# Fool-Yang/AlphaSnake-Zero

Measured on AMD Instinct MI355X. Metric: self-play env-steps/sec (11x11, 4 snakes, 50 MCTS sims), higher is better.
Workload: dtype f32 (tower convolutions: each f32 operand split into f16 hi + lo, 3 f16 MFMAs per product, f32 accumulate)

## Files before the change

### __graft_entry__.py

```python
import os
import subprocess
import sys

REPO = os.path.dirname(os.path.abspath(__file__))
PKG = os.path.join(REPO, "alphasnake-zero_amd")
for p in (REPO, PKG):
    if p not in sys.path:
        sys.path.insert(0, p)


def build():
    env = dict(os.environ)
    subprocess.check_call(["make", "-C", os.path.join(PKG, "csrc"), "-j4"], env=env)
    subprocess.check_call(["make", "-C", os.path.join(REPO, "oracle")], env=env)
    import snake_engine
    snake_engine.lib()
    import utils.game, utils.mp_game_runner, utils.agent, utils.alpha_nnet
    sys.path.insert(0, os.path.join(REPO, "tools"))
    import store_hazard_scan
    if os.path.exists(os.path.join(store_hazard_scan.LLVM_BIN, "llvm-objdump")):
        r = store_hazard_scan.scan_library(snake_engine.LIB_PATH)
        if r["violations"]:
            raise RuntimeError(f"{len(r['violations'])} wide store(s) whose data registers are rewritten inside the hazard window, e.g. "
                               f"{r['violations'][0]}")
# ... 23 lines not shown
    spawned = eng.new((n,), torch.int16, 0)
    for t in range(12):
        mv = rng.randint(0, 3, size=(n, 4)).astype(np.uint8)
        eng.step(torch.as_tensor(mv, device="cuda"), spawned=spawned)
        sp = spawned.cpu().numpy()
        for g in range(n):
            if sum(games[g].g.alive[:4]) > 1:
                games[g].tic(mv[g], spawn_cell=int(sp[g]))
    out = eng.export()
    for g in range(n):
        a, b = compact_from_state(out[g]), games[g].compact()
        for k in a:
            assert np.array_equal(a[k], b[k]), (g, k)
    alive = eng.alive().cpu().numpy()
    pairs = np.argwhere(alive).astype(np.int32)
    planes, mask, key = eng.observe_all(pairs)
    ph = planes.cpu().numpy()
    for i, (g, s) in enumerate(pairs[:256]):
        assert ph[i].tobytes() == games[g].make_state(int(s)).tobytes(), (g, s)
    from snake_engine import net
    from oracle import net_ref
    ws = net.glorot_uniform_weights((21, 21, 3), blocks=4, seed=0)
    qn = net.QNet(ws, (21, 21, 3))
    assert qn.n_rect == 6 and len(pairs) >= 64 >= qn.rect_min
    q_gpu = qn.forward(planes[:64].contiguous(), mask[:64].contiguous()).cpu().numpy()
    q_cpu = net_ref.forward(ws, ph[:64])
    assert np.abs(q_gpu - q_cpu).max() <= 1e-5, np.abs(q_gpu - q_cpu).max()
    from utils.agent import Agent
    from utils.alpha_nnet import AlphaNNet
    from utils.mp_game_runner import MPGameRunner
    MPGameRunner.verbose = False
    alice = Agent(AlphaNNet(input_shape=(21, 21, 3), _weights=ws), 2, True, 8, 8, seed=1)
    gr = MPGameRunner(11, 11, 4, 1, 4, seed=2)
    gr.run(alice, max_turns=1)
    assert gr.env_steps == 4 and len(alice.records) == 16 and np.isfinite(np.array(alice.values[:16])).all()
    print(f"smoke ok: {n} games x 12 ticks + {len(pairs)} observations bit-exact vs the CPU oracle; "
          f"net |dQ| = {np.abs(q_gpu - q_cpu).max():.2e}; one MCTS root turn of 4 games ({alice._mcts.stats['net_evals']} net evals)")


if __name__ == "__main__":
    build()
    if "--smoke" in sys.argv:
        smoke()
```

### alphasnake-zero_amd/csrc/conv_split.hip

```cpp
#include "common.h"
#include "train_fold.h"
#include <stdlib.h>

typedef float f32x16 __attribute__((ext_vector_type(16)));
typedef _Float16 f16x8 __attribute__((ext_vector_type(8)));
typedef _Float16 f16x4 __attribute__((ext_vector_type(4)));
typedef __bf16 bf16x8 __attribute__((ext_vector_type(8)));
typedef unsigned uint4_t __attribute__((ext_vector_type(4)));
typedef int i32x4 __attribute__((ext_vector_type(4)));
typedef int i32x8 __attribute__((ext_vector_type(8)));
typedef short s16x2 __attribute__((ext_vector_type(2)));

template <bool BF> __device__ __forceinline__ float hs_from16(_Float16 v)
{
    if (BF) return (float)__builtin_bit_cast(__bf16, v);
    return (float)v;
}
template <bool BF> __device__ __forceinline__ _Float16 hs_to16(float v)
{
    if (BF) return __builtin_bit_cast(_Float16, (__bf16)v);
    return (_Float16)__builtin_amdgcn_fmed3f(v, -65504.f, 65504.f);
}

#define HS_C 128
// ... 34 lines not shown
    const float *wscale_inv;
    const float *scale, *shift;
    const float *res;
    float *out;
    const float *w1x1;
    float *h1;
    float s1, b1;
    int Hd, Wd, n_blk, tiles_base, tiles_rem, relu;
    int n_img_grouped;
    const float *center;
    float *stat_part;
    const uint4 *desc;
    const int *n_desc;
    const float *bg_out;
    const float *bg_in;
    const float *bg_res;
    int grow_in, grow_res;
    const float *g_y;
    const unsigned char *g_mask;
    const float *g_inv;
    const float *aff_scale, *aff_shift;
    float *amax_part;
    const unsigned char *res_mask;
};

#ifdef HS_STAMPS
__device__ unsigned long long hs_stamp_buf[16384 * 8];
#define HS_STAMP(k) if (tid == 0 && blockIdx.x < 16384) hs_stamp_buf[blockIdx.x * 8 + (k)] = __builtin_amdgcn_s_memtime();
#define HS_STAMP_REAL(k) if (tid == 0 && blockIdx.x < 16384) hs_stamp_buf[blockIdx.x * 8 + (k)] = __builtin_amdgcn_s_memrealtime();
#define HS_STAMP_HWID(k) if (tid == 0 && blockIdx.x < 16384) hs_stamp_buf[blockIdx.x * 8 + (k)] = \
        (unsigned long long)__builtin_amdgcn_s_getreg((31 << 11) | 4) | (unsigned long long)__builtin_amdgcn_s_getreg((31 << 11) | 20) << 32;
__device__ unsigned long long hs_tap_buf[2048 * 8 * 10];
#define HS_TSTAMP(c_, s_) if (tid == 0 && blockIdx.x < 2048 && (c_) < 8) hs_tap_buf[(blockIdx.x * 8 + (c_)) * 10 + (s_)] = __builtin_amdgcn_s_memtime();
extern "C" int snk_dbg_conv_tap_stamps(unsigned long long *h_out)
{
    SNK_CHECK_HIP(hipMemcpyFromSymbol(h_out, HIP_SYMBOL(hs_tap_buf), sizeof(unsigned long long) * 2048 * 8 * 10));
    return 0;
}
extern "C" int snk_dbg_conv_stamps(unsigned long long *h_out, int n_blocks)
{
    SNK_CHECK_HIP(hipMemcpyFromSymbol(h_out, HIP_SYMBOL(hs_stamp_buf), (size_t)n_blocks * 8 * sizeof(unsigned long long)));
    return 0;
}
#else
#define HS_STAMP(k)
#define HS_STAMP_REAL(k)
// ... 19 lines not shown
}
__device__ __forceinline__ uint2 mx_quant8(const f16x8 v, unsigned &sbyte)
{
    const uint4 u = __builtin_bit_cast(uint4, v);
    const float f[8] = {__builtin_bit_cast(float, u.x << 16), __builtin_bit_cast(float, u.x & 0xFFFF0000u),
                        __builtin_bit_cast(float, u.y << 16), __builtin_bit_cast(float, u.y & 0xFFFF0000u),
                        __builtin_bit_cast(float, u.z << 16), __builtin_bit_cast(float, u.z & 0xFFFF0000u),
                        __builtin_bit_cast(float, u.w << 16), __builtin_bit_cast(float, u.w & 0xFFFF0000u)};
    float m = 0.f;
#pragma unroll
    for (int j = 0; j < 8; ++j) m = fmaxf(m, fabsf(f[j]));
    m = fmaxf(m, hs_dpp(m, 0xB1));
    m = fmaxf(m, hs_dpp(m, 0x4E));
    sbyte = mx_scale_byte(m);
    const float k = mx_inv_scale(sbyte);
    return make_uint2(mx_pack4(f[0] * k, f[1] * k, f[2] * k, f[3] * k), mx_pack4(f[4] * k, f[5] * k, f[6] * k, f[7] * k));
}
template <int NI, int MODE, bool SPLIT, int IO16, bool RECT, bool BF = false, bool MX = false, bool PK = false>
__device__ __forceinline__ void hs_block(const ConvHsArgs &p, unsigned char *smem, const int img, const int tile0, const int ntile,
                                         const int ry0, const int rx0, const int rh, const int rw, const unsigned bbox,
                                         const int part, const int parts, const int imgB = 0, const int ryB = 0, const int rxB = 0,
                                         const unsigned bboxB = 0u, const int nB = 0)
{
    static_assert(!PK || (RECT && SPLIT && IO16 == 0 && (MODE == 1 || MODE == 2)), "the packed form exists for the float32-accurate sub-rectangle layers only");
    static_assert(IO16 == 0 || !SPLIT, "f16 activations only exist in the reduced-precision form");
    static_assert(!BF || (IO16 & 1), "the bf16 form reads bf16 activations");
    static_assert(!MX || BF, "the mxfp8 form reads bf16 activations");
    constexpr bool IN16 = (IO16 & 1) != 0, OUT16 = (IO16 & 2) != 0;
    constexpr bool STATS = MODE == 4 || MODE == 6 || MODE == 9, GSTATS = MODE == 5 || MODE == 7 || MODE == 8 || MODE == 10, BARE = STATS || GSTATS;
    constexpr bool RESMASK = MODE == 8 || MODE == 10, AMAX = MODE == 4 || MODE == 9;
    constexpr bool AFF = MODE == 6 || MODE == 9, GAFF = MODE == 7 || MODE == 10, NORES = MODE == 7;
    static_assert(!(AFF || GAFF || RESMASK) || (SPLIT && IO16 == 0 && !RECT), "the deferred batch norm exists in the training step's float32 form only");
    constexpr bool K32 = IN16;
    constexpr int RING = K32 ? HS_RING16 : HS_RING, AHEAD = K32 ? HS_AHEAD16 : HS_AHEAD;
    constexpr bool TWO = SPLIT || K32;
    constexpr int KC = MX ? 64 : K32 ? 32 : HS_KC, NCHUNK = HS_C / KC;
    constexpr int NST = K32 ? HS_NST16 : HS_NST, BUFB = K32 ? HS_BUF16 : (PK ? HS_NPB_PK : HS_NPB) * HS_LDP;
    constexpr int PIECE = K32 ? 8 : 4;
    constexpr int MXR0_ = 9 * NI > 4 * NST ? (9 * NI - 4 * NST) / 2 : 0;
    constexpr int MXR0 = MXR0_ > HS_XLOAD_TAP * NI ? MXR0_ : HS_XLOAD_TAP * NI, MXT1 = (MXR0 + 2 * NST + NI - 1) / NI;
    constexpr int MXR1 = 9 * NI - 2 * NST > MXT1 * NI ? 9 * NI - 2 * NST : MXT1 * NI;
    constexpr bool MXIN = MX && 9 * NI >= 4 * NST && MXT1 <= 8 && MXR1 + 2 * NST <= 9 * NI;
    static_assert(!MXIN || (MXR0 >= HS_XLOAD_TAP * NI && MXR0 + 2 * NST <= MXT1 * NI), "MX staging: a half is written before it is loaded");
    constexpr bool P8 = IN16 && OUT16;
    const bool has_res = NORES ? false : RESMASK ? true : (MODE == 0 || GSTATS) ? p.res != nullptr : (MODE == 2 || MODE == 3);
    const bool has_head = MODE == 0 ? p.w1x1 != nullptr : MODE == 3;
    const bool has_out = MODE == 0 ? p.out != nullptr : MODE != 3;
// ... 567 lines not shown
            }
            v.x = fmaxf(v.x, relu_floor); v.y = fmaxf(v.y, relu_floor); v.z = fmaxf(v.z, relu_floor); v.w = fmaxf(v.w, relu_floor);
            if (STATS && off[pass & 1][j] >= 0) {
                const float ex = v.x - cen4.x, ey = v.y - cen4.y, ez = v.z - cen4.z, ew = v.w - cen4.w;
                st_s.x += ex; st_s.y += ey; st_s.z += ez; st_s.w += ew;
                st_q.x += ex * ex; st_q.y += ey * ey; st_q.z += ez * ez; st_q.w += ew * ew;
                if (AMAX) {
                    st_m.x = fmaxf(st_m.x, fabsf(ex)); st_m.y = fmaxf(st_m.y, fabsf(ey));
                    st_m.z = fmaxf(st_m.z, fabsf(ez)); st_m.w = fmaxf(st_m.w, fabsf(ew));
                }
            }
            if (has_out && off[pass & 1][j] >= 0) {
                if (OUT16) {
                    f16x4 o16_;
                    o16_[0] = hs_to16<BF>(v.x); o16_[1] = hs_to16<BF>(v.y); o16_[2] = hs_to16<BF>(v.z); o16_[3] = hs_to16<BF>(v.w);
                    *(f16x4 *)((_Float16 *)p.out + obase + off[pass & 1][j]) = o16_;
                } else *(float4 *)(p.out + obase + off[pass & 1][j]) = v;
            }
            if (has_head) {
                float d_ = (v.x * wh.x + v.y * wh.y) + (v.z * wh.z + v.w * wh.w);
                d_ += hs_dpp(d_, 0xB1); d_ += hs_dpp(d_, 0x4E); d_ += hs_dpp(d_, 0x141); d_ += hs_dpp(d_, 0x140);
                d_ += __shfl_xor(d_, 16, 64);
                if (cq == 0 && off[pass & 1][j] >= 0)
                    p.h1[(long)img * HWc + off[pass & 1][j] / HS_C] = fmaxf(__builtin_fmaf(d_, p.s1, p.b1), 0.f);
            }
        }
    }
#undef HS_ROWS
#undef HS_EPI_PREP
    if (BARE) {
        __syncthreads();
        float4 *R = (float4 *)smem;
        R[rr0 * 32 + cq] = st_s;
        R[(8 + rr0) * 32 + cq] = st_q;
        if (AMAX) R[(16 + rr0) * 32 + cq] = st_m;
        __syncthreads();
        if (AMAX && rr0 == 2 && p.amax_part) {
            float4 t = R[16 * 32 + cq];
#pragma unroll
            for (int r = 1; r < 8; ++r) {
                const float4 u = R[(16 + r) * 32 + cq];
                t.x = fmaxf(t.x, u.x); t.y = fmaxf(t.y, u.y); t.z = fmaxf(t.z, u.z); t.w = fmaxf(t.w, u.w);
            }
            *(float4 *)(p.amax_part + (size_t)blockIdx.x * HS_C + 4 * cq) = t;
        }
        if (rr0 < 2) {
            float4 t = R[(8 * rr0) * 32 + cq];
#pragma unroll
            for (int r = 1; r < 8; ++r) { const float4 u = R[(8 * rr0 + r) * 32 + cq]; t.x += u.x; t.y += u.y; t.z += u.z; t.w += u.w; }
            *(float4 *)(p.stat_part + (size_t)blockIdx.x * 256 + rr0 * 128 + 4 * cq) = t;
        }
    }
    if (PK && p.bg_out) {
        const float invF = 1.0f / (float)p.Wd;
        for (int s = 0; s < 2; ++s) {
            const int sm = s ? 0 : m0, sn = s ? nB : nA;
            if (sn == 0) continue;
            const int q_lo = (sm * HWc + HW - 1) / HW, q_hi = ((sm + sn) * HWc + HW - 1) / HW;
            const int fy = s ? ryB : cy0, fx = s ? rxB : cx0;
            float *ob = p.out + (long)(s ? imgB : img) * HWc * HS_C;
            for (int q = q_lo + rr0; q < q_hi; q += 8) {
                const int y_ = (int)(((float)q + 0.5f) * invF), x_ = q - y_ * p.Wd;
                if (y_ >= fy && y_ < fy + rh && x_ >= fx && x_ < fx + rw) continue;
                const int o_ = (y_ * p.Wd + x_) * HS_C + 4 * cq;
                *(float4 *)(ob + o_) = *(const float4 *)(p.bg_out + o_);
            }
        }
    } else if (RECT && p.bg_out) {
        const float invF = 1.0f / (float)p.Wd;
        for (int q = part * 8 + rr0; q < HWc; q += 8 * parts) {
            const int y_ = (int)(((float)q + 0.5f) * invF), x_ = q - y_ * p.Wd;
            if (y_ >= cy0 && y_ < cy0 + rh && x_ >= cx0 && x_ < cx0 + rw) continue;
            const int o_ = (y_ * p.Wd + x_) * HS_C + 4 * cq;
            if (OUT16) *(f16x4 *)((_Float16 *)p.out + (long)img * HWc * HS_C + o_) = *(const f16x4 *)((const _Float16 *)p.bg_out + o_);
            else *(float4 *)(p.out + (long)img * HWc * HS_C + o_) = *(const float4 *)(p.bg_out + o_);
        }
// ... 957 lines not shown
}

extern "C" int snk_conv3x3_bn_f16s_rect_pack(const float *d_x, const void *d_wS, const float *d_scale, const float *d_shift,
                                             const float *d_residual, float *d_out, const void *d_desc, const int *d_count,
                                             const float *d_bg_in, int grow_in, const float *d_bg_res, int grow_res,
                                             const float *d_bg_out, int n_images, int height, int width, void *stream)
{
    SNK_REQUIRE(grow_in >= 0 && grow_in < 128 && grow_res >= 0 && grow_res < 128, "snk_conv3x3_bn_f16s_rect_pack: grow_in %d, grow_res %d", grow_in, grow_res);
    SNK_REQUIRE(d_x && d_wS && d_scale && d_shift && d_out && d_desc && d_count, "snk_conv3x3_bn_f16s_rect_pack: NULL argument");
    SNK_REQUIRE(d_out != d_x, "snk_conv3x3_bn_f16s_rect_pack: in-place convolution is not possible");
    const long md = rect_pack_max_desc(n_images, height, width);
    SNK_REQUIRE(md >= 0 && md < (1l << 31) && (long)n_images * height * width * HS_C < (1l << 31), "snk_conv3x3_bn_f16s_rect_pack: bad shape %d x %d x %d",
                n_images, height, width);
    if (n_images == 0) return 0;
    ConvHsArgs a = {d_x, (const f16x8 *)d_wS, (const float *)((const _Float16 *)d_wS + HS_WS_ELEMS), d_scale, d_shift,
                    d_residual, d_out, nullptr, nullptr, 0.f, 0.f, height, width, 1, 0, 0, 1, 0, nullptr, nullptr,
                    (const uint4 *)d_desc, d_count, d_bg_out, d_bg_in, d_residual ? d_bg_res : nullptr, grow_in, grow_res, nullptr, nullptr, nullptr};
    if (d_residual) k_conv3x3_f16s_rectp<2><<<(int)(md / 2), 256, 0, (hipStream_t)stream>>>(a);
    else k_conv3x3_f16s_rectp<1><<<(int)(md / 2), 256, 0, (hipStream_t)stream>>>(a);
    SNK_CHECK_HIP(hipGetLastError());
    return 0;
}

extern "C" int snk_conv3x3_bn_f16_act16_rect(const void *d_x16, const void *d_wS, const float *d_scale, const float *d_shift,
                                             const void *d_residual16, void *d_out16, const void *d_desc, const int *d_count,
                                             const void *d_bg_in16, int grow_in, const void *d_bg_res16, int grow_res,
                                             const void *d_bg_out16, int n_images, int height, int width, void *stream)
{
    return conv_f16s_rect_launch((const float *)d_x16, d_wS, d_scale, d_shift, (const float *)d_residual16, (float *)d_out16, d_desc,
                                 d_count, (const float *)d_bg_in16, grow_in, (const float *)d_bg_res16, grow_res,
                                 (const float *)d_bg_out16, n_images, height, width, true, stream);
}

extern "C" int snk_conv3x3_bn_bf16_act16_rect(const void *d_x16, const void *d_wS, const float *d_scale, const float *d_shift,
                                              const void *d_residual16, void *d_out16, const void *d_desc, const int *d_count,
                                              const void *d_bg_in16, int grow_in, const void *d_bg_res16, int grow_res,
                                              const void *d_bg_out16, int n_images, int height, int width, void *stream)
{
    return conv_f16s_rect_launch((const float *)d_x16, d_wS, d_scale, d_shift, (const float *)d_residual16, (float *)d_out16, d_desc,
                                 d_count, (const float *)d_bg_in16, grow_in, (const float *)d_bg_res16, grow_res,
                                 (const float *)d_bg_out16, n_images, height, width, true, stream, true);
}

extern "C" int snk_conv3x3_bn_f16s(const float *d_x, const void *d_wS, const float *d_scale, const float *d_shift,
                                   const float *d_residual, float *d_out, int n_images, int height, int width, int relu,
                                   void *stream)
// ... 221 lines not shown
```

### alphasnake-zero_amd/snake_engine/_lib.py

```python
import ctypes as C
import os

_HERE = os.path.dirname(os.path.abspath(__file__))
LIB_PATH = os.environ.get("SNK_LIB_PATH") or os.path.join(_HERE, "libsnake_engine.so")

MAX_SNAKES, MAX_CELLS, MAX_NODES = 8, 361, 384
ABI_VERSION = 113


class EngineError(RuntimeError):
    pass


class SnkGameState(C.Structure):
    _fields_ = [
        ("H", C.c_int32), ("W", C.c_int32), ("S", C.c_int32), ("uid", C.c_uint32),
        ("alive", C.c_uint8 * MAX_SNAKES),
        ("health", C.c_int16 * MAX_SNAKES),
        ("length", C.c_int16 * MAX_SNAKES),
        ("dir", C.c_uint8 * MAX_SNAKES),
        ("nodes", (C.c_int16 * MAX_NODES) * MAX_SNAKES),
        ("food", C.c_uint8 * MAX_CELLS),
        ("rewards", C.c_int8 * MAX_SNAKES),
        ("counters", C.c_int32 * 6),
# ... 35 lines not shown
    "snk_conv3x3_bn_bf16_act16_head": (i32, [vp, vp, vp, vp, vp, vp, C.c_float, C.c_float, vp, i32, i32, i32, vp]),
    "snk_conv_rect_max_blocks_act16": (C.c_long, [i32, i32, i32]),
    "snk_conv_rect_plan_act16": (i32, [vp, C.c_float, C.c_float, C.c_float, i32, i32, i32, i32, C.POINTER(i32), vp, vp, vp, vp]),
    "snk_conv3x3_bn_bf16_act16": (i32, [vp, vp, vp, vp, vp, vp, i32, i32, i32, i32, i32, vp]),
    "snk_conv3x3_bn_bf16_act16_rect": (i32, [vp, vp, vp, vp, vp, vp, vp, vp, vp, i32, vp, i32, vp, i32, i32, i32, vp]),
    "snk_stem_conv_bn_relu_bf16out": (i32, [vp, vp, vp, vp, vp, i32, i32, i32, vp]),
    "snk_stem_conv_bn_relu_bf16out_rect": (i32, [vp, vp, vp, vp, vp, vp, i32, i32, i32, i32, vp]),
    "snk_conv3x3_prepare_weights_mxfp8": (i32, [vp, vp, vp]),
    "snk_conv3x3_bn_mxfp8_act16": (i32, [vp, vp, vp, vp, vp, vp, i32, i32, i32, i32, i32, vp]),
    "snk_conv3x3_bn_mxfp8_act16_rect": (i32, [vp, vp, vp, vp, vp, vp, vp, vp, vp, i32, vp, i32, vp, i32, i32, i32, vp]),
    "snk_conv3x3_bn_mxfp8_act16_head": (i32, [vp, vp, vp, vp, vp, vp, C.c_float, C.c_float, vp, i32, i32, i32, vp]),
    "snk_mxfp8_quantize_bf16": (i32, [vp, i32, vp, vp, vp]),
    "snk_conv3x3_prepare_weights_winograd": (i32, [vp, vp, vp]),
    "snk_conv3x3_bn_f32_winograd": (i32, [vp, vp, vp, vp, vp, vp, i32, i32, i32, i32, vp]),
    "snk_conv3x3_prepare_weights_f16s": (i32, [vp, vp, C.c_float, vp]),
    "snk_conv3x3_bn_f16s": (i32, [vp, vp, vp, vp, vp, vp, i32, i32, i32, i32, vp]),
    "snk_conv3x3_bn_f16": (i32, [vp, vp, vp, vp, vp, vp, i32, i32, i32, i32, vp]),
    "snk_conv_rect_max_blocks": (C.c_long, [i32, i32, i32]),
    "snk_conv_rect_plan": (i32, [vp, C.c_float, C.c_float, C.c_float, i32, i32, i32, i32, C.POINTER(i32), vp, vp, vp, vp]),
    "snk_conv_rect_pack_max_desc": (C.c_long, [i32, i32, i32]),
    "snk_conv_rect_plan_pack": (i32, [vp, C.c_float, C.c_float, C.c_float, i32, i32, i32, i32, C.POINTER(i32), vp, vp, vp, vp, vp]),
    "snk_conv_rect_plan_pack_host": (i32, [vp, i32, i32, i32, i32, vp, vp]),
    "snk_conv3x3_bn_f16s_rect_pack": (i32, [vp, vp, vp, vp, vp, vp, vp, vp, vp, i32, vp, i32, vp, i32, i32, i32, vp]),
    "snk_stem_conv_bn_relu_f32_rect": (i32, [vp, vp, vp, vp, vp, vp, i32, i32, i32, i32, vp]),
    "snk_stem_conv_bn_relu_f16out_rect": (i32, [vp, vp, vp, vp, vp, vp, i32, i32, i32, i32, vp]),
    "snk_conv3x3_bn_f16_act16_rect": (i32, [vp, vp, vp, vp, vp, vp, vp, vp, vp, i32, vp, i32, vp, i32, i32, i32, vp]),
    "snk_conv3x3_bn_f16s_rect": (i32, [vp, vp, vp, vp, vp, vp, vp, vp, vp, i32, vp, i32, vp, i32, i32, i32, vp]),
    "snk_conv3x3_bn_f16s_head": (i32, [vp, vp, vp, vp, vp, vp, vp, C.c_float, C.c_float, vp, i32, i32, i32, vp]),
    "snk_conv3x3_bn_f16_act16": (i32, [vp, vp, vp, vp, vp, vp, i32, i32, i32, i32, i32, vp]),
    "snk_stem_conv_bn_relu_f16out": (i32, [vp, vp, vp, vp, vp, i32, i32, i32, vp]),
    "snk_head_dense_f32": (i32, [vp, vp, vp, vp, vp, vp, vp, i32, i32, i32, vp]),
    "snk_stem_conv_bn_relu_f32": (i32, [vp, vp, vp, vp, vp, i32, i32, i32, vp]),
    "snk_tt_create": (i32, [C.POINTER(vp), u64, i32]),
    "snk_tt_destroy": (i32, [vp]),
    "snk_tt_clear": (i32, [vp, vp]),
    "snk_tt_status_sync": (i32, [vp, C.POINTER(C.c_int64), C.POINTER(C.c_int64), C.POINTER(i32)]),
    "snk_tt_rebuild_sync": (i32, [vp, u64, i32, i32]),
    "snk_tt_lookup_insert": (i32, [vp, vp, vp, i32, i32, i32, vp, vp, vp]),
    "snk_tt_find": (i32, [vp, vp, i32, i32, i32, vp, vp, vp]),
    "snk_tt_set_priors": (i32, [vp, vp, vp, i32, vp, vp, vp]),
    "snk_tt_read_q": (i32, [vp, vp, i32, i32, vp, vp]),
    "snk_mcts_select": (i32, [vp, vp, i32, C.c_float, vp, vp, C.c_int64, u64, C.c_uint32, C.c_uint32, vp, vp, vp, vp, vp, vp, i32, vp, vp]),
    "snk_mcts_gather_rows": (i32, [vp, i32, vp, vp, vp, vp, vp]),
    "snk_mcts_row_active": (i32, [vp, vp, i32, i32, vp, vp]),
    "snk_mcts_retire": (i32, [vp, vp, vp, i32, i32, vp, vp, vp]),
    "snk_mcts_backup": (i32, [vp, vp, i32, vp, vp, vp, vp, vp, i32, i32, vp, vp]),
# ... 86 lines not shown
```

### alphasnake-zero_amd/snake_engine/net.py

```python
import ctypes as C
import math
import os

import numpy as np
import torch

from ._lib import lib, check, EngineError

BN_EPS = 1e-3
K_FILTERS = 128
F16S_WEIGHT_BYTES = 9 * 128 * 128 * 4 + 32
F16S_TAIL_OFFSET = 9 * 128 * 128 * 4
F16S_FLAG_OFFSET = F16S_TAIL_OFFSET + 16


def glorot_uniform_weights(input_shape, blocks=4, seed=0):
    g = torch.Generator().manual_seed(seed)
    h, w, c = input_shape
    k = K_FILTERS

    def glorot(shape, fan_in, fan_out):
        lim = math.sqrt(6.0 / (fan_in + fan_out))
        return ((torch.rand(shape, generator=g, dtype=torch.float32) * 2 - 1) * lim).numpy()

# ... 70 lines not shown
    return count


class QNet:
    def __init__(self, weights, input_shape, device=None, max_chunk=4096):
        if not torch.cuda.is_available():
            raise EngineError("snake_engine.QNet needs an MI355X; there is no CPU fallback")
        self.L = lib()
        self.device = torch.device("cuda", torch.cuda.current_device() if device is None else int(device))
        self.input_shape = tuple(int(v) for v in input_shape)
        self.h, self.w, self.cin = self.input_shape
        assert self.cin == 3
        self.max_chunk = int(max_chunk)
        self._ws = None
        self.conv_timing = None
        self.clock_probe = None
        self.conv_algo = os.environ.get("SNK_CONV_ALGO", "f16s")
        if self.conv_algo not in ("f16s", "winograd", "direct", "bf16", "f16", "f16a", "mxfp8"):
            raise EngineError(f"SNK_CONV_ALGO={self.conv_algo!r}: expected f16s, winograd, direct, f16, f16a, bf16 or mxfp8")
        self.rect = self.conv_algo in ("f16s", "f16a", "bf16", "mxfp8") and os.environ.get("SNK_CONV_RECT", "1") != "0"
        self.act16 = {"f16a": torch.float16, "bf16": torch.bfloat16, "mxfp8": torch.bfloat16}.get(self.conv_algo)
        self.background = BACKGROUND_PIXEL
        self.guard_trips = 0
        self.rect_tiles = None
        self._bg = None
        self.rect_min = int(os.environ.get("SNK_CONV_RECT_MIN", "48"))
        self.rect_pack = os.environ.get("SNK_CONV_RECT_PACK", "1") != "0"
        self.n_streams = int(os.environ.get("SNK_NET_STREAMS", "1"))
        self._side = None
        self._guard = None
        self.set_weights(weights)

    def set_weights(self, weights):
        self.weights = [np.ascontiguousarray(w, np.float32) for w in weights]
        self.blocks = n_blocks_of(self.weights)
        dev = self.device
        t = [torch.as_tensor(w, device=dev) for w in self.weights]

        def fold(g, b, m, v):
            sc = g / torch.sqrt(v + BN_EPS)
            return sc.contiguous(), (b - m * sc).contiguous()
        self.stem_w = t[0].contiguous()
        self.stem_sc, self.stem_sh = fold(*t[1:5])
        self.conv_wT, self.conv_sc, self.conv_sh = [], [], []
        st = torch.cuda.current_stream().cuda_stream
        self.conv_x_scale = activation_scales(self.weights)
# ... 24 lines not shown
            elif self.conv_algo == "winograd":
                wT = torch.empty(16 * 128 * 128, dtype=torch.float32, device=dev)
                check(self.L.snk_conv3x3_prepare_weights_winograd(t[base].contiguous().data_ptr(), wT.data_ptr(), st))
            else:
                wT = torch.empty(9 * 128 * 128, dtype=torch.float32, device=dev)
                check(self.L.snk_conv3x3_prepare_weights(t[base].contiguous().data_ptr(), wT.data_ptr(), st))
            if self._wimg is not None and self.conv_algo not in ("bf16", "mxfp8"):
                check(self.L.snk_conv3x3_f16s_set_guard_word(wT.data_ptr(), self._guard[0].data_ptr(), st))
            sc, sh = fold(*t[base + 1:base + 5])
            self.conv_wT.append(wT); self.conv_sc.append(sc); self.conv_sh.append(sh)
        base = 5 + 10 * self.blocks
        self.head_w = t[base].reshape(128).contiguous()
        hs, hb = fold(*t[base + 1:base + 5])
        self.head_s, self.head_b = float(hs.item()), float(hb.item())
        self.fc1_w, self.fc1_b = t[base + 5].contiguous(), t[base + 6].contiguous()
        self.fc2_w, self.fc2_b = t[base + 7].contiguous(), t[base + 8].contiguous()
        self.calibrated = False
        self._bg = None
        n_layers = 2 * self.blocks
        self.n_rect = rect_layer_count(self.h, self.w, n_layers) if self.rect else 0
        if self.rect and "SNK_CONV_RECT_LAYERS" in os.environ:
            self.n_rect = max(0, min(int(os.environ["SNK_CONV_RECT_LAYERS"]), n_layers - 1))
        self.rect_fill = rect_fill_plan(self.n_rect)
        torch.cuda.current_stream().synchronize()

    def get_weights(self):
        return [w.copy() for w in self.weights]

    def _tail(self, i, dtype):
        return self.conv_wT[i][F16S_TAIL_OFFSET:F16S_TAIL_OFFSET + 32].view(dtype)

    def set_x_scale(self, i, scale):
        m, _ = math.frexp(scale)
        assert scale > 0 and m == 0.5, f"x_scale {scale} is not a power of two"
        self.conv_x_scale[i] = float(scale)
        t = self._tail(i, torch.float32)
        t[2] = float(scale)
        t[3] = 1.0 / float(scale)
        self._bg = None

    def range_flags(self, clear=True):
        if self._wimg is None:
            return []
        flags = self._wimg[:, F16S_FLAG_OFFSET:F16S_FLAG_OFFSET + 4].contiguous().view(torch.int32).reshape(-1)
        self._flags_host.copy_(flags, non_blocking=True)
        torch.cuda.current_stream().synchronize()
# ... 166 lines not shown
            if blk == self.blocks - 1:
                conv(2 * blk + 1, t1, cur, last, False)
            else:
                conv(2 * blk + 1, t1, cur, t2, True)
                cur, t2 = t2, cur
        mk = None if mask is None else mask[s0:s0 + m]
        if fused_head:
            check(L.snk_head_dense_f32(h1.data_ptr(), self.fc1_w.data_ptr(), self.fc1_b.data_ptr(), self.fc2_w.data_ptr(),
                                       self.fc2_b.data_ptr(), 0 if mk is None else mk.data_ptr(), out[s0:s0 + m].data_ptr(), m, h, w, st))
            return
        check(L.snk_head_f32(last.data_ptr(), self.head_w.data_ptr(), self.head_s, self.head_b,
                             self.fc1_w.data_ptr(), self.fc1_b.data_ptr(), self.fc2_w.data_ptr(), self.fc2_b.data_ptr(),
                             0 if mk is None else mk.data_ptr(), out[s0:s0 + m].data_ptr(), m, h, w, st))

    def _forward_chunk(self, planes, mask, out, s0, m, k):
        if self.clock_probe is not None:
            self.clock_probe.launch()
        if self.act16 is not None and self.blocks > 0:
            return self._forward_chunk_f16a(planes, mask, out, s0, m, k)
        st = torch.cuda.current_stream().cuda_stream
        L, h, w = self.L, self.h, self.w
        a, b, c = self._workspace(m, k)
        x = planes[s0:s0 + m]
        plan = self._rect_plan(x, m, k, st) if self._use_rect(m) else None
        if plan is not None and self.n_rect >= 2:
            check(L.snk_stem_conv_bn_relu_f32_rect(x.data_ptr(), self.stem_w.data_ptr(), self.stem_sc.data_ptr(),
                                                   self.stem_sh.data_ptr(), a.data_ptr(), plan[3].data_ptr(), 1, m, h, w, st))
        else:
            check(L.snk_stem_conv_bn_relu_f32(x.data_ptr(), self.stem_w.data_ptr(), self.stem_sc.data_ptr(),
                                              self.stem_sh.data_ptr(), a.data_ptr(), m, h, w, st))
        cur, t1, t2 = a, b, c
        fused_head = self.conv_algo == "f16s" and self.blocks > 0 and self._head_fits()
        for blk in range(self.blocks):
            i0, i1 = 2 * blk, 2 * blk + 1
            self._conv(i0, cur, None, t1, m, st, plan=plan)
            if fused_head and blk == self.blocks - 1:
                h1 = self._h1_workspace(m, k)
                self._conv(i1, t1, cur, None, m, st, h1=h1)
                mk = None if mask is None else mask[s0:s0 + m]
                check(L.snk_head_dense_f32(h1.data_ptr(), self.fc1_w.data_ptr(), self.fc1_b.data_ptr(), self.fc2_w.data_ptr(),
                                           self.fc2_b.data_ptr(), 0 if mk is None else mk.data_ptr(), out[s0:s0 + m].data_ptr(),
                                           m, h, w, st))
                return
            self._conv(i1, t1, cur, t2, m, st, plan=plan)
            cur, t2 = t2, cur
        mk = None if mask is None else mask[s0:s0 + m]
        check(L.snk_head_f32(cur.data_ptr(), self.head_w.data_ptr(), self.head_s, self.head_b,
                             self.fc1_w.data_ptr(), self.fc1_b.data_ptr(), self.fc2_w.data_ptr(), self.fc2_b.data_ptr(),
                             0 if mk is None else mk.data_ptr(), out[s0:s0 + m].data_ptr(), m, h, w, st))

    def _head_fits(self):
        return 4 * (self.h * self.w + 128) * 4 <= 64 * 1024

    def _h1_workspace(self, n, k=0):
        key = ("h1", k)
        if key not in self._ws or self._ws[key].shape[0] < n:
            self._ws[key] = torch.empty((n, self.h * self.w), dtype=torch.float32, device=self.device)
        return self._ws[key]

    def backgrounds(self):
        if self._bg is None:
            m, st = 1, torch.cuda.current_stream().cuda_stream
            a16 = self.act16 is not None
            dt = self.act16 if a16 else torch.float32
            blank = torch.tensor(self.background, dtype=torch.float32, device=self.device).repeat(1, self.h, self.w, 1).contiguous()
            bufs = [torch.empty((1, self.h, self.w, 128), dtype=dt, device=self.device) for _ in range(3)]
            stem = self._fn16()[0] if a16 else self.L.snk_stem_conv_bn_relu_f32
            check(stem(blank.data_ptr(), self.stem_w.data_ptr(), self.stem_sc.data_ptr(), self.stem_sh.data_ptr(),
                       bufs[0].data_ptr(), m, self.h, self.w, st))
            bg = torch.empty((1 + self.n_rect, self.h, self.w, 128), dtype=dt, device=self.device)
            bg[0].copy_(bufs[0][0])
            cur, t1, t2 = bufs
            tm, self.conv_timing = self.conv_timing, None

            def conv(i, x, res, out):
                if a16:
                    check(self._fn16()[2](x.data_ptr(), self.conv_wT[i].data_ptr(), self.conv_sc[i].data_ptr(),
                                          self.conv_sh[i].data_ptr(), None if res is None else res.data_ptr(),
                                          out.data_ptr(), 1, m, self.h, self.w, 1, st))
                else:
                    self._conv(i, x, res, out, m, st)
            for i in range(self.n_rect):
                if i % 2 == 0:
                    conv(i, cur, None, t1)
                    bg[1 + i].copy_(t1[0])
                else:
                    conv(i, t1, cur, t2)
                    bg[1 + i].copy_(t2[0])
                    cur, t2 = t2, cur
            self.conv_timing = tm
            self._bg = bg
        return self._bg

    def _rect_args(self, i, plan, res):
        desc, counts, bg = plan[:3]
        return (desc[i].data_ptr(), counts[i].data_ptr(), bg[i].data_ptr(), i + 1,
                None if res is None else bg[i - 1].data_ptr(), i, bg[1 + i].data_ptr() if self.rect_fill[i] else None)

    def _use_rect(self, m):
        return self.n_rect > 0 and m >= self.rect_min

    def _rect_plan(self, x, m, k, st):
        bg = self.backgrounds()
        a16 = self.act16 is not None
        pack = not a16 and self.rect_pack and m * self.h * self.w * 128 < 2 ** 31
        mb = int(self.L.snk_conv_rect_pack_max_desc(m, self.h, self.w)) if pack else -1
        if mb < 0:
            pack = False
            mb = int((self.L.snk_conv_rect_max_blocks_act16 if a16 else self.L.snk_conv_rect_max_blocks)(m, self.h, self.w))
        if mb < 0:
            raise EngineError(f"sub-rectangle convolution: shape {m} x {self.h} x {self.w} not supported")
        key = ("rect", k)
        ws = None if self._ws is None else self._ws.get(key)
        if ws is None or ws[0].shape[0] != self.n_rect or ws[0].shape[1] < mb or ws[2].shape[0] < m:
            ws = (torch.empty((self.n_rect, mb, 4), dtype=torch.int32, device=self.device),
                  torch.zeros((self.n_rect, 2), dtype=torch.int32, device=self.device),
                  torch.empty((m,), dtype=torch.int32, device=self.device),
                  torch.empty((self.n_rect, m), dtype=torch.int32, device=self.device))
            if self._ws is None:
                self._ws = {}
            self._ws[key] = ws
        desc, counts, bbox, order = ws
        if self.rect_tiles is not None:
            counts = torch.zeros((self.n_rect, 2), dtype=torch.int32, device=self.device)
            self.rect_tiles.append((m, counts))
        grow = (C.c_int * self.n_rect)(*[i + 2 for i in range(self.n_rect)])
        desc_m = desc if desc.shape[1] == mb else desc.view(-1)[:self.n_rect * mb * 4].view(self.n_rect, mb, 4)
        b0, b1, b2 = self.background
        if pack:
            check(self.L.snk_conv_rect_plan_pack(x.data_ptr(), b0, b1, b2, m, self.h, self.w, self.n_rect, grow, bbox.data_ptr(),
                                                 desc_m.data_ptr(), counts.data_ptr(), order.data_ptr(), st))
            return desc_m, counts, bg, bbox, True
        check((self.L.snk_conv_rect_plan_act16 if a16 else self.L.snk_conv_rect_plan)(
            x.data_ptr(), b0, b1, b2, m, self.h, self.w, self.n_rect, grow, bbox.data_ptr(), desc_m.data_ptr(), counts.data_ptr(), st))
        return desc_m, counts, bg, bbox, False

    def _conv(self, i, x, res, out, m, st, h1=None, plan=None):
        tm = self.conv_timing
        if tm is not None:
            e0, e1 = torch.cuda.Event(enable_timing=True), torch.cuda.Event(enable_timing=True)
            e0.record(torch.cuda.current_stream())
        if plan is not None and i < self.n_rect and h1 is None:
            conv_rect = self.L.snk_conv3x3_bn_f16s_rect_pack if plan[4] else self.L.snk_conv3x3_bn_f16s_rect
            check(conv_rect(x.data_ptr(), self.conv_wT[i].data_ptr(), self.conv_sc[i].data_ptr(),
                            self.conv_sh[i].data_ptr(), None if res is None else res.data_ptr(),
                            out.data_ptr(), *self._rect_args(i, plan, res), m, self.h, self.w, st))
            if tm is not None:
                e1.record(torch.cuda.current_stream())
                tm.append((e0, e1, 2.0 * m * self.h * self.w * 9 * 128 * 128))
            return
        if h1 is not None:
            check(self.L.snk_conv3x3_bn_f16s_head(x.data_ptr(), self.conv_wT[i].data_ptr(), self.conv_sc[i].data_ptr(),
                                                  self.conv_sh[i].data_ptr(), None if res is None else res.data_ptr(),
                                                  None if out is None else out.data_ptr(), self.head_w.data_ptr(),
                                                  self.head_s, self.head_b, h1.data_ptr(), m, self.h, self.w, st))
            if tm is not None:
                e1.record(torch.cuda.current_stream())
                tm.append((e0, e1, 2.0 * m * self.h * self.w * 9 * 128 * 128))
            return
        fn = {"winograd": self.L.snk_conv3x3_bn_f32_winograd,
              "f16s": self.L.snk_conv3x3_bn_f16s, "f16": self.L.snk_conv3x3_bn_f16}.get(
            self.conv_algo, self.L.snk_conv3x3_bn_f32)
        check(fn(x.data_ptr(), self.conv_wT[i].data_ptr(), self.conv_sc[i].data_ptr(),
                 self.conv_sh[i].data_ptr(), None if res is None else res.data_ptr(),
                 out.data_ptr(), m, self.h, self.w, 1, st))
# ... 28 lines not shown
```

### include/snake_engine.h

```cpp
#ifndef SNAKE_ENGINE_H
#define SNAKE_ENGINE_H

#include <stdint.h>

#ifdef __cplusplus
extern "C" {
#endif

#define SNK_MAX_SNAKES 8
#define SNK_MAX_CELLS 361
#define SNK_MAX_NODES 384

typedef struct snk_engine snk_engine;

typedef struct {
    int32_t H, W, S;
    uint32_t uid;
    uint8_t alive[SNK_MAX_SNAKES];
    int16_t health[SNK_MAX_SNAKES];
    int16_t length[SNK_MAX_SNAKES];
    uint8_t dir[SNK_MAX_SNAKES];
    int16_t nodes[SNK_MAX_SNAKES][SNK_MAX_NODES];
    uint8_t food[SNK_MAX_CELLS];
    int8_t rewards[SNK_MAX_SNAKES];
// ... 75 lines not shown
long snk_conv_rect_max_blocks_act16(int n_images, int height, int width);
int snk_conv_rect_plan_act16(const float *d_planes, float b0, float b1, float b2, int n_images, int height, int width,
                             int n_layers, const int *grow, void *d_bbox, void *d_desc, int *d_counts, void *stream);
int snk_stem_conv_bn_relu_f16out_rect(const float *d_x, const float *d_w, const float *d_scale, const float *d_shift,
                                      void *d_out16, const void *d_bbox, int grow, int n_images, int height, int width,
                                      void *stream);
int snk_conv3x3_bn_f16_act16_rect(const void *d_x16, const void *d_wS, const float *d_scale, const float *d_shift,
                                  const void *d_residual16, void *d_out16, const void *d_desc, const int *d_count,
                                  const void *d_bg_in16, int grow_in, const void *d_bg_res16, int grow_res,
                                  const void *d_bg_out16, int n_images, int height, int width, void *stream);
int snk_conv3x3_bn_f16s_rect(const float *d_x, const void *d_wS, const float *d_scale, const float *d_shift,
                             const float *d_residual, float *d_out, const void *d_desc, const int *d_count,
                             const float *d_bg_in, int grow_in, const float *d_bg_res, int grow_res,
                             const float *d_bg_out, int n_images, int height, int width, void *stream);
long snk_conv_rect_pack_max_desc(int n_images, int height, int width);
int snk_conv_rect_plan_pack(const float *d_planes, float b0, float b1, float b2, int n_images, int height, int width,
                            int n_layers, const int *grow, void *d_bbox, void *d_desc, int *d_counts, void *d_order, void *stream);
int snk_conv_rect_plan_pack_host(const unsigned *h_bbox, int n_images, int height, int width, int grow,
                                 unsigned *h_desc, int *h_counts);
int snk_conv3x3_bn_f16s_rect_pack(const float *d_x, const void *d_wS, const float *d_scale, const float *d_shift,
                                  const float *d_residual, float *d_out, const void *d_desc, const int *d_count,
                                  const float *d_bg_in, int grow_in, const float *d_bg_res, int grow_res,
                                  const float *d_bg_out, int n_images, int height, int width, void *stream);
int snk_conv3x3_bn_f16s_head(const float *d_x, const void *d_wS, const float *d_scale, const float *d_shift,
                             const float *d_residual, float *d_out, const float *d_w1x1, float bn_scale,
                             float bn_shift, float *d_h1, int n_images, int height, int width, void *stream);
int snk_conv3x3_prepare_weights_f16_act16(const float *d_w_hwio, void *d_wS, void *stream);
int snk_conv3x3_bn_f16_act16(const void *d_x16, const void *d_wS, const float *d_scale, const float *d_shift,
                             const void *d_residual16, void *d_out, int out_f16, int n_images, int height, int width,
                             int relu, void *stream);
int snk_stem_conv_bn_relu_f16out(const float *d_x, const float *d_w, const float *d_scale, const float *d_shift,
                                 void *d_out16, int n_images, int height, int width, void *stream);
int snk_conv3x3_prepare_weights_bf16(const float *d_w_hwio, void *d_wS, void *stream);
int snk_conv3x3_bn_bf16_act16(const void *d_x16, const void *d_wS, const float *d_scale, const float *d_shift,
                              const void *d_residual16, void *d_out, int out_bf16, int n_images, int height, int width,
                              int relu, void *stream);
int snk_conv3x3_bn_bf16_act16_rect(const void *d_x16, const void *d_wS, const float *d_scale, const float *d_shift,
                                   const void *d_residual16, void *d_out16, const void *d_desc, const int *d_count,
                                   const void *d_bg_in16, int grow_in, const void *d_bg_res16, int grow_res,
                                   const void *d_bg_out16, int n_images, int height, int width, void *stream);
int snk_conv3x3_bn_f16_act16_head(const void *d_x16, const void *d_wS, const float *d_scale, const float *d_shift,
                                  const void *d_residual16, const float *d_w1x1, float bn_scale, float bn_shift,
                                  float *d_h1, int n_images, int height, int width, void *stream);
int snk_conv3x3_bn_bf16_act16_head(const void *d_x16, const void *d_wS, const float *d_scale, const float *d_shift,
                                   const void *d_residual16, const float *d_w1x1, float bn_scale, float bn_shift,
                                   float *d_h1, int n_images, int height, int width, void *stream);
// ... 169 lines not shown
```

Before: 959.6.

## Extend packed sub-rectangle convolution to the last two tower layers and fused head

```diff
diff --git a/__graft_entry__.py b/__graft_entry__.py
--- a/__graft_entry__.py
+++ b/__graft_entry__.py
@@ -69,7 +69,7 @@
     from oracle import net_ref
     ws = net.glorot_uniform_weights((21, 21, 3), blocks=4, seed=0)
     qn = net.QNet(ws, (21, 21, 3))
-    assert qn.n_rect == 6 and len(pairs) >= 64 >= qn.rect_min
+    assert qn.n_rect == 6 and qn.n_rect_pack == 8 and len(pairs) >= 64 >= qn.rect_min
     q_gpu = qn.forward(planes[:64].contiguous(), mask[:64].contiguous()).cpu().numpy()
     q_cpu = net_ref.forward(ws, ph[:64])
     assert np.abs(q_gpu - q_cpu).max() <= 1e-5, np.abs(q_gpu - q_cpu).max()
diff --git a/alphasnake-zero_amd/csrc/conv_split.hip b/alphasnake-zero_amd/csrc/conv_split.hip
--- a/alphasnake-zero_amd/csrc/conv_split.hip
+++ b/alphasnake-zero_amd/csrc/conv_split.hip
@@ -80,6 +80,7 @@
     const float *aff_scale, *aff_shift;
     float *amax_part;
     const unsigned char *res_mask;
+    const float *bg_h1;
 };
 
 #ifdef HS_STAMPS
@@ -145,7 +146,7 @@
                                          const int part, const int parts, const int imgB = 0, const int ryB = 0, const int rxB = 0,
                                          const unsigned bboxB = 0u, const int nB = 0)
 {
-    static_assert(!PK || (RECT && SPLIT && IO16 == 0 && (MODE == 1 || MODE == 2)), "the packed form exists for the float32-accurate sub-rectangle layers only");
+    static_assert(!PK || (RECT && SPLIT && IO16 == 0 && (MODE == 1 || MODE == 2 || MODE == 3)), "the packed form exists for the float32-accurate sub-rectangle layers only");
     static_assert(IO16 == 0 || !SPLIT, "f16 activations only exist in the reduced-precision form");
     static_assert(!BF || (IO16 & 1), "the bf16 form reads bf16 activations");
     static_assert(!MX || BF, "the mxfp8 form reads bf16 activations");
@@ -759,7 +760,7 @@
                 d_ += hs_dpp(d_, 0xB1); d_ += hs_dpp(d_, 0x4E); d_ += hs_dpp(d_, 0x141); d_ += hs_dpp(d_, 0x140);
                 d_ += __shfl_xor(d_, 16, 64);
                 if (cq == 0 && off[pass & 1][j] >= 0)
-                    p.h1[(long)img * HWc + off[pass & 1][j] / HS_C] = fmaxf(__builtin_fmaf(d_, p.s1, p.b1), 0.f);
+                    p.h1[(PK ? 0l : (long)img * HWc) + off[pass & 1][j] / HS_C] = fmaxf(__builtin_fmaf(d_, p.s1, p.b1), 0.f);
             }
         }
     }
@@ -788,7 +789,21 @@
             *(float4 *)(p.stat_part + (size_t)blockIdx.x * 256 + rr0 * 128 + 4 * cq) = t;
         }
     }
-    if (PK && p.bg_out) {
+    if (PK && MODE == 3) {
+        const float invF = 1.0f / (float)p.Wd;
+        for (int s = 0; s < 2; ++s) {
+            const int sm = s ? 0 : m0, sn = s ? nB : nA;
+            if (sn == 0) continue;
+            const int q_lo = (sm * HWc + HW - 1) / HW, q_hi = ((sm + sn) * HWc + HW - 1) / HW;
+            const int fy = s ? ryB : cy0, fx = s ? rxB : cx0;
+            float *hb = p.h1 + (long)(s ? imgB : img) * HWc;
+            for (int q = q_lo + tid; q < q_hi; q += 256) {
+                const int y_ = (int)(((float)q + 0.5f) * invF), x_ = q - y_ * p.Wd;
+                if (y_ >= fy && y_ < fy + rh && x_ >= fx && x_ < fx + rw) continue;
+                hb[q] = p.bg_h1[q];
+            }
+        }
+    } else if (PK && p.bg_out) {
         const float invF = 1.0f / (float)p.Wd;
         for (int s = 0; s < 2; ++s) {
             const int sm = s ? 0 : m0, sn = s ? nB : nA;
@@ -1792,6 +1807,28 @@
     return 0;
 }
 
+extern "C" int snk_conv3x3_bn_f16s_rect_pack_head(const float *d_x, const void *d_wS, const float *d_scale, const float *d_shift,
+                                                  const float *d_residual, const float *d_w1x1, float bn_scale, float bn_shift,
+                                                  float *d_h1, const void *d_desc, const int *d_count, const float *d_bg_in,
+                                                  int grow_in, const float *d_bg_res, int grow_res, const float *d_bg_h1,
+                                                  int n_images, int height, int width, void *stream)
+{
+    SNK_REQUIRE(grow_in >= 0 && grow_in < 128 && grow_res >= 0 && grow_res < 128, "snk_conv3x3_bn_f16s_rect_pack_head: grow_in %d, grow_res %d", grow_in, grow_res);
+    SNK_REQUIRE(d_x && d_wS && d_scale && d_shift && d_residual && d_w1x1 && d_h1 && d_desc && d_count && d_bg_h1,
+                "snk_conv3x3_bn_f16s_rect_pack_head: NULL argument");
+    const long md = rect_pack_max_desc(n_images, height, width);
+    SNK_REQUIRE(md >= 0 && md < (1l << 31) && (long)n_images * height * width * HS_C < (1l << 31), "snk_conv3x3_bn_f16s_rect_pack_head: bad shape %d x %d x %d",
+                n_images, height, width);
+    if (n_images == 0) return 0;
+    ConvHsArgs a = {d_x, (const f16x8 *)d_wS, (const float *)((const _Float16 *)d_wS + HS_WS_ELEMS), d_scale, d_shift,
+                    d_residual, nullptr, d_w1x1, d_h1, bn_scale, bn_shift, height, width, 1, 0, 0, 1, 0, nullptr, nullptr,
+                    (const uint4 *)d_desc, d_count, nullptr, d_bg_in, d_bg_res, grow_in, grow_res, nullptr, nullptr, nullptr};
+    a.bg_h1 = d_bg_h1;
+    k_conv3x3_f16s_rectp<3><<<(int)(md / 2), 256, 0, (hipStream_t)stream>>>(a);
+    SNK_CHECK_HIP(hipGetLastError());
+    return 0;
+}
+
 extern "C" int snk_conv3x3_bn_f16_act16_rect(const void *d_x16, const void *d_wS, const float *d_scale, const float *d_shift,
                                              const void *d_residual16, void *d_out16, const void *d_desc, const int *d_count,
                                              const void *d_bg_in16, int grow_in, const void *d_bg_res16, int grow_res,
diff --git a/alphasnake-zero_amd/snake_engine/_lib.py b/alphasnake-zero_amd/snake_engine/_lib.py
--- a/alphasnake-zero_amd/snake_engine/_lib.py
+++ b/alphasnake-zero_amd/snake_engine/_lib.py
@@ -81,6 +81,8 @@
     "snk_conv_rect_plan_pack": (i32, [vp, C.c_float, C.c_float, C.c_float, i32, i32, i32, i32, C.POINTER(i32), vp, vp, vp, vp, vp]),
     "snk_conv_rect_plan_pack_host": (i32, [vp, i32, i32, i32, i32, vp, vp]),
     "snk_conv3x3_bn_f16s_rect_pack": (i32, [vp, vp, vp, vp, vp, vp, vp, vp, vp, i32, vp, i32, vp, i32, i32, i32, vp]),
+    "snk_conv3x3_bn_f16s_rect_pack_head": (i32, [vp, vp, vp, vp, vp, vp, C.c_float, C.c_float, vp, vp, vp, vp, i32, vp, i32, vp,
+                                                 i32, i32, i32, vp]),
     "snk_stem_conv_bn_relu_f32_rect": (i32, [vp, vp, vp, vp, vp, vp, i32, i32, i32, i32, vp]),
     "snk_stem_conv_bn_relu_f16out_rect": (i32, [vp, vp, vp, vp, vp, vp, i32, i32, i32, i32, vp]),
     "snk_conv3x3_bn_f16_act16_rect": (i32, [vp, vp, vp, vp, vp, vp, vp, vp, vp, i32, vp, i32, vp, i32, i32, i32, vp]),
diff --git a/alphasnake-zero_amd/snake_engine/net.py b/alphasnake-zero_amd/snake_engine/net.py
--- a/alphasnake-zero_amd/snake_engine/net.py
+++ b/alphasnake-zero_amd/snake_engine/net.py
@@ -116,6 +116,7 @@
         self.act16 = {"f16a": torch.float16, "bf16": torch.bfloat16, "mxfp8": torch.bfloat16}.get(self.conv_algo)
         self.background = BACKGROUND_PIXEL
         self.guard_trips = 0
+        self.rect_tiles_all = None
         self.rect_tiles = None
         self._bg = None
         self.rect_min = int(os.environ.get("SNK_CONV_RECT_MIN", "48"))
@@ -186,6 +187,11 @@
         if self.rect and "SNK_CONV_RECT_LAYERS" in os.environ:
             self.n_rect = max(0, min(int(os.environ["SNK_CONV_RECT_LAYERS"]), n_layers - 1))
         self.rect_fill = rect_fill_plan(self.n_rect)
+        self.n_rect_pack = self.n_rect
+        if self.n_rect > 0 and self.conv_algo == "f16s" and self.rect_pack:
+            cap = n_layers if self._head_fits() else n_layers - 1
+            self.n_rect_pack = max(0, min(int(os.environ.get("SNK_CONV_RECT_LAYERS", n_layers)), cap))
+        self.rect_fill_pack = rect_fill_plan(self.n_rect_pack)
         torch.cuda.current_stream().synchronize()
 
     def get_weights(self):
@@ -398,8 +404,8 @@
         L, h, w = self.L, self.h, self.w
         a, b, c = self._workspace(m, k)
         x = planes[s0:s0 + m]
-        plan = self._rect_plan(x, m, k, st) if self._use_rect(m) else None
-        if plan is not None and self.n_rect >= 2:
+        plan = self._rect_plan(x, m, k, st, all_layers=True) if self._use_rect(m) else None
+        if plan is not None and plan[6] >= 2:
             check(L.snk_stem_conv_bn_relu_f32_rect(x.data_ptr(), self.stem_w.data_ptr(), self.stem_sc.data_ptr(),
                                                    self.stem_sh.data_ptr(), a.data_ptr(), plan[3].data_ptr(), 1, m, h, w, st))
         else:
@@ -412,7 +418,7 @@
             self._conv(i0, cur, None, t1, m, st, plan=plan)
             if fused_head and blk == self.blocks - 1:
                 h1 = self._h1_workspace(m, k)
-                self._conv(i1, t1, cur, None, m, st, h1=h1)
+                self._conv(i1, t1, cur, None, m, st, h1=h1, plan=plan)
                 mk = None if mask is None else mask[s0:s0 + m]
                 check(L.snk_head_dense_f32(h1.data_ptr(), self.fc1_w.data_ptr(), self.fc1_b.data_ptr(), self.fc2_w.data_ptr(),
                                            self.fc2_b.data_ptr(), 0 if mk is None else mk.data_ptr(), out[s0:s0 + m].data_ptr(),
@@ -444,7 +450,9 @@
             stem = self._fn16()[0] if a16 else self.L.snk_stem_conv_bn_relu_f32
             check(stem(blank.data_ptr(), self.stem_w.data_ptr(), self.stem_sc.data_ptr(), self.stem_sh.data_ptr(),
                        bufs[0].data_ptr(), m, self.h, self.w, st))
-            bg = torch.empty((1 + self.n_rect, self.h, self.w, 128), dtype=dt, device=self.device)
+            n_layers = 2 * self.blocks
+            n_bg = self.n_rect if a16 else max(self.n_rect, min(self.n_rect_pack, n_layers - 1))
+            bg = torch.empty((1 + n_bg, self.h, self.w, 128), dtype=dt, device=self.device)
             bg[0].copy_(bufs[0][0])
             cur, t1, t2 = bufs
             tm, self.conv_timing = self.conv_timing, None
@@ -456,7 +464,7 @@
                                           out.data_ptr(), 1, m, self.h, self.w, 1, st))
                 else:
                     self._conv(i, x, res, out, m, st)
-            for i in range(self.n_rect):
+            for i in range(n_bg):
                 if i % 2 == 0:
                     conv(i, cur, None, t1)
                     bg[1 + i].copy_(t1[0])
@@ -464,20 +472,29 @@
                     conv(i, t1, cur, t2)
                     bg[1 + i].copy_(t2[0])
                     cur, t2 = t2, cur
+            bg_h1 = None
+            if not a16 and self.n_rect_pack == n_layers and n_layers > 0:
+                bg_h1 = torch.empty((self.h * self.w,), dtype=torch.float32, device=self.device)
+                self._conv(n_layers - 1, t1, cur, None, m, st, h1=bg_h1)
             self.conv_timing = tm
-            self._bg = bg
+            self._bg_all = (bg, bg_h1)
+            self._bg = bg[:1 + self.n_rect]
         return self._bg
+
+    def _backgrounds_all(self):
+        self.backgrounds()
+        return self._bg_all
 
     def _rect_args(self, i, plan, res):
         desc, counts, bg = plan[:3]
         return (desc[i].data_ptr(), counts[i].data_ptr(), bg[i].data_ptr(), i + 1,
-                None if res is None else bg[i - 1].data_ptr(), i, bg[1 + i].data_ptr() if self.rect_fill[i] else None)
+                None if res is None else bg[i - 1].data_ptr(), i, bg[1 + i].data_ptr() if plan[5][i] else None)
 
     def _use_rect(self, m):
         return self.n_rect > 0 and m >= self.rect_min
 
-    def _rect_plan(self, x, m, k, st):
-        bg = self.backgrounds()
+    def _rect_plan(self, x, m, k, st, all_layers=False):
+        bg = self._backgrounds_all()[0]
         a16 = self.act16 is not None
         pack = not a16 and self.rect_pack and m * self.h * self.w * 128 < 2 ** 31
         mb = int(self.L.snk_conv_rect_pack_max_desc(m, self.h, self.w)) if pack else -1
@@ -486,37 +503,53 @@
             mb = int((self.L.snk_conv_rect_max_blocks_act16 if a16 else self.L.snk_conv_rect_max_blocks)(m, self.h, self.w))
         if mb < 0:
             raise EngineError(f"sub-rectangle convolution: shape {m} x {self.h} x {self.w} not supported")
+        n = self.n_rect_pack if all_layers and pack else self.n_rect
+        fill = self.rect_fill_pack if all_layers and pack else self.rect_fill
+        if n == 0:
+            return None
         key = ("rect", k)
         ws = None if self._ws is None else self._ws.get(key)
-        if ws is None or ws[0].shape[0] != self.n_rect or ws[0].shape[1] < mb or ws[2].shape[0] < m:
-            ws = (torch.empty((self.n_rect, mb, 4), dtype=torch.int32, device=self.device),
-                  torch.zeros((self.n_rect, 2), dtype=torch.int32, device=self.device),
+        if ws is None or ws[0].shape[0] != n or ws[0].shape[1] < mb or ws[2].shape[0] < m:
+            ws = (torch.empty((n, mb, 4), dtype=torch.int32, device=self.device),
+                  torch.zeros((n, 2), dtype=torch.int32, device=self.device),
                   torch.empty((m,), dtype=torch.int32, device=self.device),
-                  torch.empty((self.n_rect, m), dtype=torch.int32, device=self.device))
+                  torch.empty((n, m), dtype=torch.int32, device=self.device))
             if self._ws is None:
                 self._ws = {}
             self._ws[key] = ws
         desc, counts, bbox, order = ws
         if self.rect_tiles is not None:
-            counts = torch.zeros((self.n_rect, 2), dtype=torch.int32, device=self.device)
-            self.rect_tiles.append((m, counts))
-        grow = (C.c_int * self.n_rect)(*[i + 2 for i in range(self.n_rect)])
-        desc_m = desc if desc.shape[1] == mb else desc.view(-1)[:self.n_rect * mb * 4].view(self.n_rect, mb, 4)
+            counts = torch.zeros((n, 2), dtype=torch.int32, device=self.device)
+            self.rect_tiles.append((m, counts[:self.n_rect]))
+            if self.rect_tiles_all is not None:
+                self.rect_tiles_all.append((m, counts))
+        grow = (C.c_int * n)(*[i + 2 for i in range(n)])
+        desc_m = desc if desc.shape[1] == mb else desc.view(-1)[:n * mb * 4].view(n, mb, 4)
         b0, b1, b2 = self.background
         if pack:
-            check(self.L.snk_conv_rect_plan_pack(x.data_ptr(), b0, b1, b2, m, self.h, self.w, self.n_rect, grow, bbox.data_ptr(),
+            check(self.L.snk_conv_rect_plan_pack(x.data_ptr(), b0, b1, b2, m, self.h, self.w, n, grow, bbox.data_ptr(),
                                                  desc_m.data_ptr(), counts.data_ptr(), order.data_ptr(), st))
-            return desc_m, counts, bg, bbox, True
+            return desc_m, counts, bg, bbox, True, fill, n
         check((self.L.snk_conv_rect_plan_act16 if a16 else self.L.snk_conv_rect_plan)(
-            x.data_ptr(), b0, b1, b2, m, self.h, self.w, self.n_rect, grow, bbox.data_ptr(), desc_m.data_ptr(), counts.data_ptr(), st))
-        return desc_m, counts, bg, bbox, False
+            x.data_ptr(), b0, b1, b2, m, self.h, self.w, n, grow, bbox.data_ptr(), desc_m.data_ptr(), counts.data_ptr(), st))
+        return desc_m, counts, bg, bbox, False, fill, n
 
     def _conv(self, i, x, res, out, m, st, h1=None, plan=None):
         tm = self.conv_timing
         if tm is not None:
             e0, e1 = torch.cuda.Event(enable_timing=True), torch.cuda.Event(enable_timing=True)
             e0.record(torch.cuda.current_stream())
-        if plan is not None and i < self.n_rect and h1 is None:
+        if plan is not None and i < plan[6] and h1 is not None:
+            desc, counts, bg = plan[:3]
+            check(self.L.snk_conv3x3_bn_f16s_rect_pack_head(
+                x.data_ptr(), self.conv_wT[i].data_ptr(), self.conv_sc[i].data_ptr(), self.conv_sh[i].data_ptr(), res.data_ptr(),
+                self.head_w.data_ptr(), self.head_s, self.head_b, h1.data_ptr(), desc[i].data_ptr(), counts[i].data_ptr(),
+                bg[i].data_ptr(), i + 1, bg[i - 1].data_ptr(), i, self._backgrounds_all()[1].data_ptr(), m, self.h, self.w, st))
+            if tm is not None:
+                e1.record(torch.cuda.current_stream())
+                tm.append((e0, e1, 2.0 * m * self.h * self.w * 9 * 128 * 128))
+            return
+        if plan is not None and i < plan[6] and h1 is None:
             conv_rect = self.L.snk_conv3x3_bn_f16s_rect_pack if plan[4] else self.L.snk_conv3x3_bn_f16s_rect
             check(conv_rect(x.data_ptr(), self.conv_wT[i].data_ptr(), self.conv_sc[i].data_ptr(),
                             self.conv_sh[i].data_ptr(), None if res is None else res.data_ptr(),
diff --git a/include/snake_engine.h b/include/snake_engine.h
--- a/include/snake_engine.h
+++ b/include/snake_engine.h
@@ -121,6 +121,11 @@
                                   const float *d_residual, float *d_out, const void *d_desc, const int *d_count,
                                   const float *d_bg_in, int grow_in, const float *d_bg_res, int grow_res,
                                   const float *d_bg_out, int n_images, int height, int width, void *stream);
+int snk_conv3x3_bn_f16s_rect_pack_head(const float *d_x, const void *d_wS, const float *d_scale, const float *d_shift,
+                                       const float *d_residual, const float *d_w1x1, float bn_scale, float bn_shift,
+                                       float *d_h1, const void *d_desc, const int *d_count, const float *d_bg_in,
+                                       int grow_in, const float *d_bg_res, int grow_res, const float *d_bg_h1,
+                                       int n_images, int height, int width, void *stream);
 int snk_conv3x3_bn_f16s_head(const float *d_x, const void *d_wS, const float *d_scale, const float *d_shift,
                              const float *d_residual, float *d_out, const float *d_w1x1, float bn_scale,
                              float bn_shift, float *d_h1, int n_images, int height, int width, void *stream);
```

Result: no change. 962.1, median of 6 (+0.3%).
